# MihailMihov/simd-raytracer

Hardware: AMD Instinct MI355X
Metric: Mrays/s (intersect invocations per second), hw09/scene5 dragon 1920x1080 1spp (higher is better)
Workload: dtype f32; 1 GPU; BASELINE configs[1]: scenes/hw09/scene5.crtscene 1920x1080 1spp max_ray_depth=5 (primary + shadow + reflection rays), kd_tree_simd_accel semantics; rays_per_frame=2726485, primary_rays=2073600, parallelism=bucket-tiles x1

## Files before the change

### simd-raytracer_amd/csrc/api.hip

```cpp
#include <hip/hip_runtime.h>

#include <algorithm>
#include <cmath>
#include <cstdio>
#include <cstdlib>
#include <cstring>
#include <mutex>
#include <new>

#include "kernels.hpp"
#include "stream.hpp"
#include "repack.hpp"
#include "occluded.hpp"
#include "build.hpp"

namespace rtk {

static thread_local std::string g_last_error;
void set_error(const std::string &msg) { g_last_error = msg; }

namespace {

int fail(int code, const std::string &msg) { set_error(msg); return code; }

int hip_fail(hipError_t e, const char *what) {
    set_error(std::string(what) + ": " + hipGetErrorString(e));
    return RTK_ERR_HIP;
}

#define RTK_HIP(call)                                        \
    do {                                                     \
        const hipError_t e_ = (call);                        \
        if (e_ != hipSuccess) return hip_fail(e_, #call);    \
    } while (0)

template <typename T>
int upload(const std::vector<T> &src, T **dst) {
    *dst = nullptr;
    const size_t bytes = (src.empty() ? 1 : src.size()) * sizeof(T);
    RTK_HIP(hipMalloc(reinterpret_cast<void **>(dst), bytes));
    if (!src.empty()) RTK_HIP(hipMemcpy(*dst, src.data(), src.size() * sizeof(T), hipMemcpyHostToDevice));
    return RTK_OK;
}

}
}

struct rtk_knobs {
    uint32_t slice_min_tris = rtk::kSliceMinTrisDefault;
    bool shadow_exit = true;
    bool skip_unlit_shadow = true;
    bool bundle_cull = true;
    bool auto_trials = true;
    bool cost_feedback = true;
    unsigned resort_every = 16;
    uint32_t light_cycles = 140000u;
    uint32_t order_floor_cycles = 20000u;
    bool batch_scalar_surv = false;
    bool stream_scalar_surv = true;
    bool repack = true;
    bool raster_tiles = true;
    int repack_skip_bits = 6;
    bool repack_full_bounds = false;
    int repack_skip_bits2 = 14;
    bool repack_dirs3 = false;
    int repack_trace = -1;
    size_t group8_below = 9000;
    int stream_node_factor = 0;
    int stream_deep_level = 99, stream_deep_mode = RTK_TRACE_AUTO;
    uint32_t auto_min_lanes = 12;
    int stream_sort_from = -1;
    bool stream_debug = false;
    bool stream_side = true;
    int stream_lanes = 4;
    int stream_slices = 0;
    int stream_batch = 0;
    int stream_mem_gb = 96;
    int stream_side_below = 2;
    bool first_frame_prior = true;
    bool fast_occluders = true;
    bool traversal_fast = false;

    static rtk_knobs from_env() {
        rtk_knobs k;
        auto geti = [](const char *name, long &out) { const char *e = std::getenv(name); if (!e || !*e) return false; out = std::atol(e); return true; };
        long v;
        if (geti("RTK_SLICE_MIN_TRIS", v) && v > 0) k.slice_min_tris = uint32_t(v);
        if (geti("RTK_SHADOW_EARLY_EXIT", v)) k.shadow_exit = v != 0;
        if (geti("RTK_SKIP_UNLIT_SHADOW", v)) k.skip_unlit_shadow = v != 0;
        if (geti("RTK_BUNDLE_CULL", v)) k.bundle_cull = v != 0;
        if (geti("RTK_AUTO_TRIALS", v)) k.auto_trials = v != 0;
        if (geti("RTK_COST_FEEDBACK", v)) k.cost_feedback = v != 0;
        if (geti("RTK_COST_RESORT_EVERY", v) && v > 0) k.resort_every = unsigned(v);
        if (geti("RTK_LIGHT_BELOW_CYCLES", v) && v >= 0) k.light_cycles = uint32_t(v);
        if (geti("RTK_ORDER_FLOOR_CYCLES", v) && v >= 0) k.order_floor_cycles = uint32_t(v);
        if (geti("RTK_REPACK", v)) k.repack = v != 0;
        if (geti("RTK_RASTER_TILES", v)) k.raster_tiles = v != 0;
        if (geti("RTK_REPACK_FULL_BOUNDS", v)) k.repack_full_bounds = v != 0;
        if (geti("RTK_REPACK_SKIP_BITS2", v) && v >= 0 && v <= 22) k.repack_skip_bits2 = int(v);
        if (geti("RTK_REPACK_DIRS3", v)) k.repack_dirs3 = v != 0;
        if (geti("RTK_REPACK_SKIP_BITS", v) && v >= 0 && v <= 14) k.repack_skip_bits = int(v);
        if (geti("RTK_STREAM_SCALAR_SURV", v)) k.stream_scalar_surv = v != 0;
        if (geti("RTK_BATCH_SCALAR_SURV", v)) k.batch_scalar_surv = v != 0;
        if (geti("RTK_REPACK_TRACE", v) && (v == RTK_TRACE_AUTO || v == RTK_TRACE_WAVE || v == RTK_TRACE_LANE)) k.repack_trace = int(v);
        if (geti("RTK_GROUP8_BELOW_BLOCKS", v) && v >= 0) k.group8_below = size_t(v);
        if (geti("RTK_STREAM_NODE_FACTOR", v) && v >= 1) k.stream_node_factor = int(v);
        if (geti("RTK_STREAM_DEEP_LEVEL", v)) k.stream_deep_level = int(v);
        if (geti("RTK_STREAM_DEEP_MODE", v)) k.stream_deep_mode = int(v);
        if (geti("RTK_AUTO_MIN_LANES", v) && v > 0 && v <= 64) k.auto_min_lanes = uint32_t(v);
        if (geti("RTK_STREAM_SORT_FROM", v)) k.stream_sort_from = int(v);
        if (geti("RTK_STREAM_DEBUG", v)) k.stream_debug = v != 0;
        if (geti("RTK_STREAM_SIDE", v)) k.stream_side = v != 0;
        if (geti("RTK_TRAVERSAL_FAST", v)) k.traversal_fast = v != 0;
        if (geti("RTK_FIRST_FRAME_PRIOR", v)) k.first_frame_prior = v != 0;
        if (geti("RTK_STREAM_SLICES", v) && (v == 0 || v == 1 || v == 2 || v == 4)) k.stream_slices = int(v);
        if (geti("RTK_STREAM_BATCH", v) && v >= 0 && v <= 4096) k.stream_batch = int(v);
        if (geti("RTK_STREAM_MEM_GB", v) && v >= 1 && v <= 256) k.stream_mem_gb = int(v);
        if (geti("RTK_FAST_OCCLUDERS", v)) k.fast_occluders = v != 0;
        if (geti("RTK_STREAM_SIDE_BELOW", v) && v >= 0) k.stream_side_below = int(v);
        if (geti("RTK_STREAM_LANES", v) && v >= 1 && v <= rtk::dev::kStreamLanes) k.stream_lanes = int(v);
        return k;
    }
// ... 1080 lines not shown
static int render_device_impl(rtk_accel *a, const rtk_render_params *p, float *d_out, hipStream_t s) {
    FrameGeom g;
    int rc = frame_geom(a, p, g);
    if (rc != RTK_OK) return rc;
    if (!d_out) return fail(RTK_ERR_INVALID, "null output buffer");
    dev::RenderArgs A;
    std::memset(&A, 0, sizeof(A));
    A.tree = tree_view(a);
    A.materials = a->d_materials; A.lights = a->d_lights;
    A.textures = a->d_textures; A.tri_uv = a->d_tri_uv; A.tex_pixels = a->d_tex_pixels;
    A.n_lights = int(a->scene.lights.size());
    A.has_refractive = a->has_refractive ? 1 : 0;
    std::memcpy(A.cam_pos, a->scene.cam_pos, sizeof(A.cam_pos));
    std::memcpy(A.cam_mat, a->scene.cam_mat, sizeof(A.cam_mat));
    std::memcpy(A.background, a->scene.background, sizeof(A.background));
    A.width = g.width; A.height = g.height;
    A.aspect = static_cast<float>(g.width) / static_cast<float>(g.height);
    const float fov_radians = static_cast<float>(p->fov_degrees * (3.14159265358979323846 / 180.0));
    A.tan_half_fov = std::tan(fov_radians / 2.0f);
    A.spp = p->spp; A.max_depth = p->max_ray_depth; A.diffuse_rays = p->diffuse_rays; A.seed = p->seed;
    A.width_f = static_cast<float>(g.width); A.height_f = static_cast<float>(g.height);
    A.spp_f = static_cast<float>(p->spp); A.gi_div_f = static_cast<float>(p->diffuse_rays + 1);
    A.sample_begin = g.sample_begin; A.sample_end = g.sample_end;
    A.shadow_bias = p->shadow_bias; A.reflection_bias = p->reflection_bias; A.refraction_bias = p->refraction_bias;
    A.bucket = g.bucket; A.tiles_x = g.tiles_x; A.tiles_y = g.tiles_y; A.n_buckets = g.n_buckets;
    A.blocks_per_bucket_side = g.blocks_side; A.buckets_per_rank = g.buckets_per_rank;
    A.rank = g.rank; A.world = g.world; A.compact = g.world > 1 ? 1 : 0; A.skew_q = g.skew_q;
    A.out = d_out; A.counters = a->d_counters;
    A.slice_min_tris = a->knobs.slice_min_tris;
    const bool forks = a->has_refractive || p->diffuse_rays > 0;
    const bool general = forks || !a->scene.textures.empty();
    A.shadow_exit = (a->knobs.shadow_exit && !a->has_refractive && p->collect_stats != 1) ? 1 : 0;
    A.skip_unlit = (a->knobs.skip_unlit_shadow && !a->has_refractive && p->collect_stats != 1) ? 1 : 0;
    A.occl_on = (a->occl_on && p->collect_stats == 0) ? 1 : 0;
    A.occl = A.tree;
    if (A.occl_on) {
        A.occl.nodes = a->d_occl_nodes; A.occl.leaves = a->d_occl_leaves; A.occl.leaves_fast = nullptr; A.occl.n_leaves = a->occl_n_leaves;
        A.occl.tris = a->d_occl_tris; A.occl.tri_ids = a->d_occl_ids;
    }
    RTK_HIP(hipMemsetAsync(a->d_counters, 0, (kCounterWords + 4) * sizeof(unsigned long long), s));
    if (g.world > 1 && g.sample_begin == 0) {
        size_t nf = size_t(g.buckets_per_rank) * g.bucket * g.bucket * 3;
        RTK_HIP(hipMemsetAsync(d_out, 0, nf * sizeof(float), s));
    }
    bool stream = p->trace_mode == RTK_TRACE_STREAM || (p->trace_mode == RTK_TRACE_AUTO && forks);
    hipEvent_t trial_start = nullptr, trial_end = nullptr;
    if (p->trace_mode == RTK_TRACE_AUTO && forks && !p->collect_stats) {
        const bool trials = a->knobs.auto_trials;
        const uint64_t tsig[3] = {(uint64_t(uint32_t(g.width)) << 32) | uint32_t(g.height), (uint64_t(uint32_t(g.rank)) << 32) | uint32_t(g.world),
                                  (uint64_t(uint32_t(p->spp)) << 32) | (uint64_t(uint32_t(p->max_ray_depth)) << 16) | uint32_t(p->diffuse_rays)};
        if (std::memcmp(tsig, a->trial_sig, sizeof(tsig)) != 0) { std::memcpy(a->trial_sig, tsig, sizeof(tsig)); a->trial_state = 0; }
        if (trials) {
            if (!a->trial_ev[0]) for (auto &e : a->trial_ev) RTK_HIP(hipEventCreate(&e));
            if (a->trial_state == 3) {
                float t_stream = 0.f, t_mega = 0.f;
                if (hipEventQuery(a->trial_ev[1]) == hipSuccess && hipEventQuery(a->trial_ev[3]) == hipSuccess &&
                    hipEventElapsedTime(&t_stream, a->trial_ev[0], a->trial_ev[1]) == hipSuccess &&
                    hipEventElapsedTime(&t_mega, a->trial_ev[2], a->trial_ev[3]) == hipSuccess)
                    a->trial_state = t_mega < t_stream ? 5 : 4;
                else (void)hipGetLastError();
            }
            switch (a->trial_state) {
                case 0: stream = true; trial_start = a->trial_ev[0]; trial_end = a->trial_ev[1]; a->trial_state = 1; break;
                case 1: stream = false; a->trial_state = 2; break;
                case 2: stream = false; trial_start = a->trial_ev[2]; trial_end = a->trial_ev[3]; a->trial_state = 3; break;
                case 5: stream = false; break;
// ... 516 lines not shown
```

### simd-raytracer_amd/csrc/kernels.hip

```cpp
#include <hip/hip_runtime.h>

#include "kernels.hpp"
#include "trace.hip.hpp"
#include "common.hip.hpp"

namespace rtk {
namespace dev {

__device__ __forceinline__ void stage_nodes(const DevNode *g_nodes, uint32_t n_nodes, DevNode *lds_nodes) {
    const float4 *src = reinterpret_cast<const float4 *>(g_nodes);
    float4 *dst = reinterpret_cast<float4 *>(lds_nodes);
    for (uint32_t i = threadIdx.x; i < n_nodes * 2u; i += blockDim.x) dst[i] = src[i];
    __syncthreads();
}

__device__ __forceinline__ void flush_stats(const Stats &st, uint32_t rays, unsigned long long *counters) {
    const uint32_t r = wave_sum(rays), h = wave_sum(st.hits), nd = wave_sum(st.nodes), bp = wave_sum(st.boxpass),
                   lv = wave_sum(st.leaves), tr = wave_sum(st.tris), pk = wave_sum(st.packets16);
    if ((threadIdx.x & 63u) == 0u) {
        atomicAdd(counters + 0, (unsigned long long)r);
        atomicAdd(counters + 2, (unsigned long long)h);
        atomicAdd(counters + 3, (unsigned long long)nd);
        atomicAdd(counters + 4, (unsigned long long)bp);
        atomicAdd(counters + 5, (unsigned long long)lv);
        atomicAdd(counters + 6, (unsigned long long)tr);
        atomicAdd(counters + 7, (unsigned long long)pk);
    }
}

template <int MODE, bool STATS, bool LDS_NODES>
__global__ __launch_bounds__(256) void k_intersect(IntersectArgs A) {
    extern __shared__ __attribute__((aligned(16))) unsigned char smem[];
    DevNode *lds_nodes = reinterpret_cast<DevNode *>(smem);
    if (LDS_NODES) stage_nodes(A.tree.nodes, A.tree.n_nodes, lds_nodes);

    const size_t slot = (size_t)blockIdx.x * blockDim.x + threadIdx.x;
// ... 32 lines not shown
            o0 = make_float4(c.t, c.u, c.v, __uint_as_float(s.tri));
            o1 = make_float4(__uint_as_float(s.mesh), s.hit_normal.x, s.hit_normal.y, s.hit_normal.z);
        } else {
            o0 = make_float4(-1.0f, 0.0f, 0.0f, __uint_as_float(kMiss));
            o1 = make_float4(__uint_as_float(kMiss), 0.0f, 0.0f, 0.0f);
        }
        float4 *out = reinterpret_cast<float4 *>(A.out + i);
        out[0] = o0;
        out[1] = o1;
    }
    if (STATS) flush_stats(st, active ? 1u : 0u, A.counters);
}


__device__ __forceinline__ bool upper_half(const V3 d, const bool sel) {
    Ray q;
    q.o = d; q.d = d; q.inv = d;
    const DirSpread S = dir_spread(q, sel);
    const float dv = S.axis == 0u ? d.x : (S.axis == 1u ? d.y : d.z);
    return sel & !(dv <= S.mid);
}
__device__ __forceinline__ uint32_t burst_part(const V3 d, const bool in, const uint32_t plog) {
    uint32_t part = 0u;
    if (plog == 0u) return part;
    if (upper_half(d, in)) part = 1u;
    if (plog >= 2u) {
#pragma unroll
        for (uint32_t h = 0u; h < 2u; ++h)
            if (upper_half(d, in & (part == h))) part |= 2u;
    }
    return part;
}

template <int SLICES>
struct ShadowBurstService {
    const RenderArgs &A;
    float4 *res;
    __device__ __forceinline__ void operator()(GroupShared *sh, const uint32_t slice) const {
        const uint32_t lane = __lane_id();
        const uint32_t hdr = (uint32_t)__builtin_amdgcn_readfirstlane((int)sh->count);
        const uint32_t plog = hdr & 0xFFu, n_jobs = hdr >> 8;
        const uint32_t first = (uint32_t)__builtin_amdgcn_readfirstlane((int)sh->first);
        const unsigned long long mask = sh->pass_mask;
        const float4 a = sh->ray_o[lane], b = sh->ray_d[lane];
        const V3 P = mk(a.x, a.y, a.z), ncos = mk(a.w, b.x, b.y);
        const bool in_burst = ((mask >> lane) & 1ull) != 0ull;
        for (;;) {
            uint32_t job = 0u;
            if (lane == 0u) job = atomicAdd(&sh->pad[0], 1u);
            job = (uint32_t)__builtin_amdgcn_readfirstlane((int)job);
            if (job >= n_jobs) break;
            const uint32_t k = first + (job >> plog);
            const uint32_t part = job & ((1u << plog) - 1u);
            const float PI_F = 3.14159265358979323846f;
            const DevLight *L = A.lights + k;
            const V3 lp = mk(L->pos[0], L->pos[1], L->pos[2]);
            V3 ld = lp - P;
            const float radius = length(ld);
            const float area = 4.0f * PI_F * radius * radius;
            ld = normalized(ld);
            const float d0 = dot(ld, ncos);
            const float cosine = (0.0f < d0) ? d0 : 0.0f;
            const float contrib = (L->intensity / area) * cosine;
            const bool mine = in_burst & (burst_part(ld, in_burst, plog) == part);
            const bool asked = mine & (0.0f < radius);
            const bool q = asked & !(A.skip_unlit != 0 && unlit_query(contrib, b.z));
            const Ray ray = make_ray(P + (A.shadow_bias * ld), ld);
            Stats st = {0, 0, 0, 0, 0, 0};
            SliceCtx sx = {nullptr, 0xFFFFFFFFu, 0u, true, 0u, group_private_bundles<SLICES>(sh, slice)};
            const float exit_t = A.shadow_exit ? radius : -1.0f;
            const Cand c = trace<RTK_TRACE_WAVE, false, false, 1>(A.tree, nullptr, ray, false, q, st, sx, kAutoMinLanes, exit_t,
                                                                  kClsHasApex | (0x100u + k), lp);
            bool clear = true;
            uint32_t fl = mine ? 2u : 0u;
            if (asked) fl |= 1u;
            if (q) clear = (c.k == kMiss) | (radius < c.t);
            res[job * 64u + lane] = make_float4(contrib, clear ? 1.0f : 0.0f, __uint_as_float(fl), 0.0f);
        }
    }
};

__device__ __forceinline__ uint32_t fresh_lane() {
    uint32_t l;
    asm volatile("v_mbcnt_lo_u32_b32 %0, -1, 0\n\tv_mbcnt_hi_u32_b32 %0, -1, %0" : "=v"(l));
    return l;
}

__device__ __forceinline__ Ray spawn_ray(const V3 o, const V3 d) {
    Ray r;
    r.o = o; r.d = d; r.inv = d;
    return r;
}

enum : int { ST_NEW_SAMPLE = 0, ST_TRACE, ST_SHADE, ST_LIGHT, ST_RETURN, ST_DONE };
enum : int { PEND_CHILD_BG = 0, PEND_CHILD_BLACK = 1, PEND_SHADOW = 2 };
enum : uint32_t { FR_REFR_A = 0, FR_REFR_B = 1, FR_DIFFUSE = 2 };

struct Frame {
    float a[12];
    uint32_t meta;
    uint32_t tri;
    uint32_t key;
};

template <int MODE, bool STATS, bool FORKS, bool LDS_NODES, int SLICES, bool PRIMED = false>
__global__ __launch_bounds__(SLICES > 1 ? 64 * SLICES : 256, SLICES == 16 ? 1 : SLICES == 8 ? 2 : (SLICES == 4 && !STATS ? RTK_G4_WAVES : 4)) void k_render(RenderArgs A) {
#ifdef RTK_DEBUG_PHASES
    const unsigned long long ph_entry = __builtin_readcyclecounter();
    const unsigned long long ph_rt0 = __builtin_amdgcn_s_memrealtime();
#endif
    if (PRIMED && blockIdx.x >= *A.n_listed) return;
    if (A.only_if != nullptr && *A.only_if == 0u) return;
    extern __shared__ __attribute__((aligned(16))) unsigned char smem[];
    DevNode *lds_nodes = reinterpret_cast<DevNode *>(smem);
    constexpr bool kStage = LDS_NODES && (MODE == RTK_TRACE_LANE || MODE == RTK_TRACE_AUTO);
    if (kStage) stage_nodes(A.tree.nodes, A.tree.n_nodes, lds_nodes);
    __shared__ GroupStorage<(SLICES > 1 ? SLICES : 1)> group_st;
    GroupShared *const group_sh = group_st.get();
    const uint32_t wave_in_wg = (uint32_t)__builtin_amdgcn_readfirstlane((int)(threadIdx.x >> 6));
    uint32_t slice = SLICES > 1 ? (wave_in_wg + blockIdx.x) % (uint32_t)SLICES : 0u;
    uint32_t gwave;
    bool light = false;
    if (PRIMED) {
        gwave = A.tile_order[blockIdx.x];
    } else if (SLICES > 1 && A.order_in != nullptr) {
        const uint32_t n_wgs = A.order_hdr[0], n_total = A.order_hdr[1];
        if (blockIdx.x >= n_wgs) return;
        const uint32_t desc = A.wg_list[blockIdx.x];
        if ((desc >> 31) == 0u) {
            gwave = desc;
        } else {
            const uint32_t idx = (desc & 0x7FFFFFFFu) + wave_in_wg;
            if (idx >= n_total) return;
            gwave = A.order_in[idx];
            light = true;
            slice = 0u;
        }
    } else {
        const uint32_t unit = SLICES > 1 ? blockIdx.x : blockIdx.x * (blockDim.x >> 6) + wave_in_wg;
        gwave = (A.order_in != nullptr && unit < A.n_units) ? A.order_in[unit] : unit;
    }
    constexpr int kParkSlots = 4;
    __shared__ __attribute__((aligned(16))) float park_lds[kParkSlots][18][64];
    float4 *const burst_res = reinterpret_cast<float4 *>(&park_lds[1][0][0]);
    constexpr uint32_t kBurstMaxJobs = SLICES > 8 ? 8u : SLICES > 1 ? (uint32_t)SLICES : 1u;
    static_assert(SLICES <= 1 || (size_t)kBurstMaxJobs * 64 * sizeof(float4) <= sizeof(float) * (kParkSlots - 1) * 18 * 64, "burst answers fit the spare parking slots");
    if (SLICES > 1 && slice != 0u) {
        group_helper_loop<SLICES>(A.tree, group_sh, slice, ShadowBurstService<SLICES>{A, burst_res});
        return;
    }
    __shared__ __attribute__((aligned(16))) float wave_bundles[4][kMaxBundles * kBundleFloats];
    SliceCtx sx = {SLICES > 1 ? group_sh : nullptr, light ? 0xFFFFFFFFu : A.slice_min_tris, 0u, true, 0u,
                   (SLICES > 1 && !light) ? group_sh->bundles : wave_bundles[wave_in_wg & 3u]};
    const uint32_t park_slot = (SLICES > 1 && !light) ? 0u : (wave_in_wg & 3u);
    const unsigned long long cost_t0 = __builtin_readcyclecounter();
    const unsigned long long real_t0 = __builtin_amdgcn_s_memrealtime();
    constexpr bool writer = true;
    const uint32_t bpb = A.blocks_per_bucket_side * A.blocks_per_bucket_side;
    const uint32_t local_bucket = gwave / bpb, sub = gwave % bpb;
    const uint32_t bucket = rank_bucket((uint32_t)A.rank, local_bucket, (uint32_t)A.world, A.skew_q);
    bool valid = bucket < A.n_buckets;
    const uint32_t bx = (bucket % A.tiles_x) * A.bucket, by = (bucket / A.tiles_x) * A.bucket;
    const uint32_t sub_x0 = (sub % A.blocks_per_bucket_side) * 8u, sub_y0 = (sub / A.blocks_per_bucket_side) * 8u;
    struct Pixel { uint32_t lx, ly, px, py; };
    const auto my_pixel = [&]() {
        const uint32_t l = fresh_lane();
        Pixel p;
        p.lx = sub_x0 + (l & 7u); p.ly = sub_y0 + (l >> 3);
        p.px = bx + p.lx; p.py = by + p.ly;
        return p;
    };
    {
        const Pixel p = my_pixel();
        valid = valid & (p.lx < A.bucket) & (p.ly < A.bucket) & (p.px < A.width) & (p.py < A.height);
    }

#ifdef RTK_DEBUG_PHASES
    const unsigned long long ph_begin = __builtin_readcyclecounter();
#endif
    const V3 background = mk(A.background[0], A.background[1], A.background[2]);
    const V3 black = mk(0.f, 0.f, 0.f);
    const float PI_F = 3.14159265358979323846f;
    const uint32_t seed_hash = pcg_hash(A.seed);

    int state = valid ? ST_NEW_SAMPLE : ST_DONE;
    int pend = PEND_CHILD_BG;
    int sample = A.sample_begin, depth = 0, light_k = 0;
    uint32_t rkey = 0;
    uint32_t nrays_wave = 0;
    bool cull = false;
    Ray ray = spawn_ray(black, mk(1.f, 1.f, 1.f));
    V3 pixel_sum = black, ret = black;
    if (A.sample_begin > 0 && valid) {
        const Pixel p = my_pixel();
        const float *o = A.out + A.out_index(local_bucket, p.lx, p.ly, p.px, p.py) * 3;
        pixel_sum = mk(o[0], o[1], o[2]);
    }
    V3 P = black, hn = black, fn = black, din = black, ncos = black, acc = black, albedo = black;
    uint32_t hit_tri = 0, hit_mat = 0;
    float shadow_max_t = 0.f, contrib = 0.f;
    bool lit_textured = false;
    Frame frames[FORKS ? kMaxRayDepth : 1];
    int fsp = 0;
    Stats st = {0, 0, 0, 0, 0, 0};
    Cand cand;
    cand.t = kFltMax; cand.u = cand.v = 0.f; cand.k = kMiss;
    bool primed = false;
    V3 mirror_apex = black;
    bool burst_done = false;
    unsigned long long burst_lanes = 0ull;
    uint32_t burst_plog_done = 0u, burst_part0 = 0u;
    uint32_t burst_nl_done = 0u;
#ifdef RTK_DEBUG_PHASES
    unsigned long long ph_first_trace = 0, ph_after_first = 0, ph_wait = 0;
    float ph_tr[6] = {0.f, 0.f, 0.f, 0.f, 0.f, 0.f}, ph_kind[6] = {0.f, 0.f, 0.f, 0.f, 0.f, 0.f};
    float ph_job[3][8] = {{0.f}}, ph_own[1] = {0.f};
#endif

    for (;;) {
        while (state != ST_TRACE && state != ST_DONE) {
            if (state == ST_NEW_SAMPLE) {
                if (sample == A.sample_end) {
                    const float inv = A.spp_f;
                    if (writer) {
                        const Pixel p = my_pixel();
                        float *o = A.out + A.out_index(local_bucket, p.lx, p.ly, p.px, p.py) * 3;
                        if (A.spp == 1 || A.sample_end != A.spp) { o[0] = pixel_sum.x; o[1] = pixel_sum.y; o[2] = pixel_sum.z; }
                        else { o[0] = pixel_sum.x / inv; o[1] = pixel_sum.y / inv; o[2] = pixel_sum.z / inv; }
                    }
                    state = ST_DONE;
                    continue;
                }
                const Pixel p = my_pixel();
                rkey = root_key(seed_hash, p.py * A.width + p.px, (uint32_t)sample);
                ray = camera_ray(A, p.px, p.py, rkey);
                mirror_apex = ray.o;
                cull = true; depth = 0; pend = PEND_CHILD_BG; fsp = 0;
                primed = PRIMED;
                state = ST_TRACE;
            } else if (state == ST_SHADE) {
                if (depth == A.max_depth) { ret = background; state = ST_RETURN; continue; }
                const DevMaterial *mat = A.materials + hit_mat;
                const int kind = mat->kind;
                if (kind == RTK_MAT_CONSTANT) {
                    ret = mk(mat->albedo[0], mat->albedo[1], mat->albedo[2]);
// ... 137 lines not shown
                        cull = false; depth = fdepth + 1; pend = PEND_CHILD_BLACK;
                        state = ST_TRACE;
                    } else {
                        P = fP; hn = fhn;
                        acc = mk(f.a[9], f.a[10], f.a[11]);
                        hit_tri = f.tri;
                        const DevShade *sh = A.tree.shade + hit_tri;
                        fn = mk(sh->fn[0], sh->fn[1], sh->fn[2]);
                        hit_mat = sh->material;
                        const DevMaterial *mat = A.materials + hit_mat;
                        albedo = mk(mat->albedo[0], mat->albedo[1], mat->albedo[2]);
                        ncos = mat->smooth ? hn : fn;
                        lit_textured = false;
                        depth = fdepth;
                        fsp -= 1;
                        light_k = 0;
                        state = ST_LIGHT;
                    }
                }
            }
        }

        const bool need = (state == ST_TRACE);
        if (__ballot(need) == 0ull) break;
        hn = black; fn = black; din = black; ret = black;
        hit_tri = 0u; hit_mat = 0u;
        constexpr bool kRootFirst = !STATS && MODE == RTK_TRACE_WAVE;
        ray.inv = mk((1.0f / ray.d.x), (1.0f / ray.d.y), (1.0f / ray.d.z));
        const float reach = albedo_reach(albedo);
        const bool unlit = (A.skip_unlit != 0) & need & (pend == PEND_SHADOW) && unlit_query(contrib, reach);
        const bool traced = need & !unlit;
        const bool in_root = kRootFirst ? enters_root(A.tree, ray, traced) : traced;
        bool burst = false;
        uint32_t burst_k = 0u, burst_plog = 0u, burst_nl = 0u;
        unsigned long long burst_mask = 0ull;
        bool elsewhere = false;
        uint32_t burst_my_part = 0u;
        if (SLICES > 1 && !STATS && !light && A.has_refractive == 0) {
            const bool sh_lane = need & (pend == PEND_SHADOW);
            burst_mask = __builtin_amdgcn_ballot_w64(sh_lane);
            if (burst_mask != 0ull) {
                burst_k = (uint32_t)__builtin_amdgcn_readlane(light_k, __builtin_ctzll(burst_mask));
                const uint32_t left = (uint32_t)A.n_lights - burst_k;
                burst_nl = left < kBurstMaxJobs ? left : kBurstMaxJobs;
                burst_plog = (burst_nl * 4u <= kBurstMaxJobs) ? 2u : (burst_nl * 2u <= kBurstMaxJobs) ? 1u : 0u;
                burst = (__builtin_amdgcn_ballot_w64(sh_lane & ((uint32_t)light_k != burst_k)) == 0ull) & (1u < (burst_nl << burst_plog));
                if (burst && A.skip_unlit != 0) {
                    bool lit = sh_lane & !unlit;
                    for (uint32_t s = 1u; s < burst_nl; ++s) {
                        const DevLight *L = A.lights + burst_k + s;
                        V3 ld = mk(L->pos[0], L->pos[1], L->pos[2]) - P;
                        const float radius = length(ld);
                        const float area = 4.0f * PI_F * radius * radius;
                        ld = normalized(ld);
                        const float d0 = dot(ld, ncos);
                        const float cosine = (0.0f < d0) ? d0 : 0.0f;
                        lit |= sh_lane & !unlit_query((L->intensity / area) * cosine, reach);
                    }
                    burst = wave_any(lit);
                }
                if (burst) burst_my_part = burst_part(ray.d, sh_lane, burst_plog);
                elsewhere = burst & sh_lane & (burst_my_part != 0u);
            }
        }
        const bool quiet = kRootFirst && !burst && !(PRIMED && wave_any(primed)) && !wave_any(in_root);
        if (quiet) {
            cand.t = kFltMax; cand.u = cand.v = 0.f; cand.k = kMiss;
            burst_done = false;
        } else {
        float *const park = &park_lds[park_slot][0][fresh_lane()];
        park[0 * 64] = pixel_sum.x; park[1 * 64] = pixel_sum.y; park[2 * 64] = pixel_sum.z;
        park[3 * 64] = acc.x; park[4 * 64] = acc.y; park[5 * 64] = acc.z;
        park[6 * 64] = albedo.x; park[7 * 64] = albedo.y; park[8 * 64] = albedo.z;
        park[9 * 64] = ncos.x; park[10 * 64] = ncos.y; park[11 * 64] = ncos.z;
        park[12 * 64] = P.x; park[13 * 64] = P.y; park[14 * 64] = P.z;
        park[15 * 64] = mirror_apex.x; park[16 * 64] = mirror_apex.y; park[17 * 64] = mirror_apex.z;
        if (PRIMED && wave_any(primed)) {
            if (need) {
                const Pixel p = my_pixel();
                const float4 pc = A.prim[A.out_index(local_bucket, p.lx, p.ly, p.px, p.py)];
                cand.t = pc.x; cand.u = pc.y; cand.v = pc.z; cand.k = __float_as_uint(pc.w);
            }
            nrays_wave -= (uint32_t)__popcll(__builtin_amdgcn_ballot_w64(need));
            primed = false;
            burst_done = false;
        } else {
#ifdef RTK_DEBUG_PHASES
            const unsigned long long tr0 = __builtin_readcyclecounter();
            if (ph_first_trace == 0) ph_first_trace = tr0;
#endif
            const float exit_t = (A.shadow_exit && pend == PEND_SHADOW) ? shadow_max_t : -1.0f;
            uint32_t cls = (uint32_t)depth;
            V3 apex = black;
            if (pend == PEND_CHILD_BG) { cls |= kClsHasApex; apex = mirror_apex; }
            if (pend == PEND_SHADOW) {
                const DevLight *L = A.lights + light_k;
                cls = kClsHasApex | (0x100u + (uint32_t)light_k + 0x40u * (uint32_t)depth);
                apex = mk(L->pos[0], L->pos[1], L->pos[2]);
            }
            if (burst) {
                const uint32_t lane = fresh_lane();
                group_sh->ray_o[lane] = make_float4(P.x, P.y, P.z, ncos.x);
                group_sh->ray_d[lane] = make_float4(ncos.y, ncos.z, reach, 0.f);
                if (lane == 0u) {
                    group_sh->pass_mask = burst_mask; group_sh->first = burst_k; group_sh->count = burst_plog | ((burst_nl << burst_plog) << 8);
                    group_sh->pad[0] = 1u;
                    uint32_t extra = GROUP_EXTRA;
                    asm volatile("" : "+v"(extra));
                    group_sh->kind = extra;
                }
                __syncthreads();
                sx.min_tris = 0xFFFFFFFFu;
            }
            cand = trace<MODE, STATS, kStage, SLICES, kRootFirst>(A.tree, lds_nodes, ray, cull, in_root & !elsewhere, st, sx, kAutoMinLanes, exit_t, cls, apex);
#ifdef RTK_DEBUG_PHASES
            const unsigned long long ph_w0 = __builtin_readcyclecounter();
#endif
            if (burst) {
                __syncthreads();
                sx.min_tris = A.slice_min_tris;
            }
#ifdef RTK_DEBUG_PHASES
            ph_wait += __builtin_readcyclecounter() - ph_w0;
            if (burst && SLICES > 1) ph_own[0] = (float)(ph_w0 - tr0);
            for (int i = 0; i < 6; ++i) if (sx.n_trace == (uint32_t)i) {
                ph_tr[i] = (float)(__builtin_readcyclecounter() - tr0);
                ph_kind[i] = burst ? 100.f + (float)burst_plog : (float)__popcll(__builtin_amdgcn_ballot_w64(in_root));
            }
#endif
            burst_done = burst; burst_lanes = burst_mask; burst_plog_done = burst_plog; burst_part0 = burst_my_part;
            burst_nl_done = burst_nl;
#ifdef RTK_DEBUG_PHASES
            sx.c_trace += __builtin_readcyclecounter() - tr0; sx.n_trace += 1u;
            if (ph_after_first == 0) ph_after_first = __builtin_readcyclecounter();
#endif
        }

        float *const unpark = &park_lds[park_slot][0][fresh_lane()];
        pixel_sum = mk(unpark[0 * 64], unpark[1 * 64], unpark[2 * 64]);
        acc = mk(unpark[3 * 64], unpark[4 * 64], unpark[5 * 64]);
        albedo = mk(unpark[6 * 64], unpark[7 * 64], unpark[8 * 64]);
        ncos = mk(unpark[9 * 64], unpark[10 * 64], unpark[11 * 64]);
        P = mk(unpark[12 * 64], unpark[13 * 64], unpark[14 * 64]);
        mirror_apex = mk(unpark[15 * 64], unpark[16 * 64], unpark[17 * 64]);
        }

        uint32_t more_rays = 0u;
        if (need) {
            const uint32_t lane = fresh_lane();
            more_rays = 1u;
            const bool hit = cand.k != kMiss;
            if (pend == PEND_SHADOW) {
                bool clear = !hit | (shadow_max_t < cand.t);
                const bool in_burst = SLICES > 1 && burst_done && ((burst_lanes >> lane) & 1ull) != 0ull;
                const uint32_t my_part = in_burst ? burst_part0 : 0u;
                if (my_part != 0u) clear = burst_res[my_part * 64u + lane].y != 0.0f;
                bool again = false;
                if (!clear && A.has_refractive) {
                    const uint32_t tri = A.tree.tri_ids[cand.k];
                    const uint32_t m = A.tree.shade[tri].material;
                    if (A.materials[m].kind == RTK_MAT_REFRACTIVE) {
                        const V3 hp = ray.o + (cand.t * ray.d);
                        ray.o = hp + (A.shadow_bias * ray.d);
                        shadow_max_t -= cand.t;
                        if (0.0f < shadow_max_t) again = true; else clear = true;
                    }
                }
                if (!again) {
                    if (clear) acc = acc + (contrib * albedo);
                    light_k += 1;
                    state = ST_LIGHT;
                    if (in_burst) {
                        const uint32_t plog = burst_plog_done;
                        for (uint32_t s = 1u; s < burst_nl_done; ++s) {
                            for (uint32_t pp = 0u; pp < (1u << plog); ++pp) {
                                const float4 res = burst_res[((s << plog) + pp) * 64u + lane];
                                const uint32_t fl = __float_as_uint(res.z);
                                if ((fl & 2u) != 0u) {
                                    if (res.y != 0.0f) acc = acc + (res.x * albedo);
                                    more_rays += fl & 1u;
                                }
                            }
                            light_k += 1;
                        }
                    }
                }
            } else if (!hit) {
                ret = (pend == PEND_CHILD_BG) ? background : black;
                state = ST_RETURN;
            } else {
                const Surface s = reconstruct(A.tree, cand);
                P = ray.o + (cand.t * ray.d);
                hn = s.hit_normal; fn = s.face_normal; din = ray.d;
                hit_tri = s.tri; hit_mat = s.material;
                if (FORKS && A.tri_uv != nullptr && A.materials[hit_mat].kind == RTK_MAT_TEXTURE)
                    albedo = sample_texture(A.textures + A.materials[hit_mat].texture, A.tri_uv + hit_tri, cand.u, cand.v, A.tex_pixels);
                state = ST_SHADE;
            }
        }
        nrays_wave += (uint32_t)__popcll(__builtin_amdgcn_ballot_w64((more_rays & 1u) != 0u)) +
                      2u * (uint32_t)__popcll(__builtin_amdgcn_ballot_w64((more_rays & 2u) != 0u)) +
                      4u * (uint32_t)__popcll(__builtin_amdgcn_ballot_w64((more_rays & 4u) != 0u)) +
                      8u * (uint32_t)__popcll(__builtin_amdgcn_ballot_w64((more_rays & 8u) != 0u));
        static_assert(kBurstMaxJobs + 1u <= 15u, "a lane's rays of one iteration fit four bits");
    }

    const uint32_t lane = fresh_lane();
#ifdef RTK_DEBUG_PHASES
    const Pixel dbg_p = my_pixel();
    const uint32_t lx = dbg_p.lx, ly = dbg_p.ly, px = dbg_p.px, py = dbg_p.py;
    if (valid && writer) {
        const unsigned long long ph_now = __builtin_readcyclecounter();
        const unsigned long long ph_rt1 = __builtin_amdgcn_s_memrealtime();
        const float vals[60] = {(float)(ph_now - ph_begin), (float)sx.c_trace, (float)sx.n_trace, (float)sx.n_steps,
                                (float)sx.n_small, (float)sx.t_small, (float)sx.c_small, (float)sx.n_big, (float)sx.t_big, (float)sx.c_big,
// ... 436 lines not shown
```

### simd-raytracer_amd/csrc/kernels.hpp

```cpp
#pragma once

#include <hip/hip_runtime.h>

#include "rtk_internal.hpp"

namespace rtk {

constexpr int kMaxRayDepth = 16;
constexpr int kRayCounterShards = 64;
constexpr int kCriticalWord = 8 + kRayCounterShards;
constexpr unsigned long long kCriticalMinTicks = 1000;
constexpr int kCounterWords = 8 + 2 * kRayCounterShards;
constexpr int kCostBins = 64;
constexpr uint32_t kSliceMinTrisDefault = 33;
constexpr size_t kMaxNodeLdsBytes = 48 * 1024;

}

#include "trace.hip.hpp"

namespace rtk {
namespace dev {

__host__ __device__ inline uint32_t rank_bucket(uint32_t rank, uint32_t local, uint32_t world, uint32_t skew_q) {
// ... 32 lines not shown
    float cam_pos[3];
    float cam_mat[9];
    float background[3];
    uint32_t width, height;
    float aspect;
    float tan_half_fov;
    int spp, max_depth, diffuse_rays;
    int sample_begin, sample_end;
    uint32_t seed;
    float shadow_bias, reflection_bias, refraction_bias;
    uint32_t bucket, tiles_x, tiles_y, n_buckets, blocks_per_bucket_side;
    uint32_t buckets_per_rank;
    uint32_t skew_q;
    int rank, world;
    uint32_t slice_min_tris;
    int compact;
    float *out;
    unsigned long long *counters;
    float4 *prim;
    uint32_t *bin_count;
    uint32_t *bin_list;
    uint32_t *tile_order;
    uint32_t *n_listed;
    uint32_t tile_cap;
    const uint32_t *only_if;
    uint32_t n_units;
    uint32_t *cost_out;
    float width_f, height_f, spp_f, gi_div_f;
    const uint32_t *order_in;
    const uint32_t *order_hdr;
    const uint32_t *wg_list;
    int shadow_exit;
    int skip_unlit;
    int occl_on;
    TreeView occl;

    __device__ __forceinline__ size_t out_index(uint32_t local_bucket, uint32_t lx, uint32_t ly, uint32_t px,
                                                uint32_t py) const {
        return compact ? (((size_t)local_bucket * bucket + ly) * bucket + lx) : ((size_t)py * width + px);
    }
};

struct AssembleArgs {
    const float *gathered;
    float *rgb;
    uint32_t width, height, bucket, tiles_x, world, buckets_per_rank, skew_q;
};

}

hipError_t launch_intersect(const dev::IntersectArgs &A, int mode, bool stats, hipStream_t s);
hipError_t launch_render(const dev::RenderArgs &A, int mode, bool stats, bool forks, hipStream_t s, unsigned n_workgroups = 0);
hipError_t launch_order_by_cost(const uint32_t *cost, uint8_t *bins , uint32_t *order, uint32_t *wg_list ,
                                uint32_t *hdr , uint32_t n, uint32_t light_below, uint32_t floor_below, uint32_t pack,
                                hipStream_t s);
hipError_t launch_block_prior(const dev::RenderArgs &A, uint8_t *cls, uint32_t *order, uint32_t *wg_list, uint32_t *hdr,
                              uint32_t *scratch, uint32_t pack, hipStream_t s);
hipError_t launch_twopass(const dev::RenderArgs &A, bool stats, bool forks, hipStream_t s);
hipError_t launch_assemble(const dev::AssembleArgs &A, hipStream_t s);
hipError_t launch_camera_rays(const dev::RenderArgs &A, int sample, rtk_ray *d_rays, hipStream_t s);
hipError_t launch_to_rgb8(const float *d_rgb, size_t n, uint8_t *d_out, hipStream_t s);

}
```

Before: 14170 Mrays/s.

## Deal shadow burst jobs per light by lit-lane counts via shared table

Reworks the shadow-burst helper protocol. The owning wave now precomputes per-light contributions and lit masks in LDS, then builds a job table where each light gets its own split count. Helper slices pick their light and partition from that table instead of using one uniform split for all lights. The aim is to spend helper jobs only on lights that have lit lanes and to balance the lanes across jobs. In exchange it adds LDS board traffic, per-lane extra light evaluations up front, and more complex job decoding.

New measurement: 14230 Mrays/s (median of 4 runs). Within noise of the previous version (+0.5%).

```diff
diff --git a/simd-raytracer_amd/csrc/api.hip b/simd-raytracer_amd/csrc/api.hip
--- a/simd-raytracer_amd/csrc/api.hip
+++ b/simd-raytracer_amd/csrc/api.hip
@@ -50,6 +50,7 @@
     uint32_t slice_min_tris = rtk::kSliceMinTrisDefault;
     bool shadow_exit = true;
     bool skip_unlit_shadow = true;
+    int burst_deal = 0;
     bool bundle_cull = true;
     bool auto_trials = true;
     bool cost_feedback = true;
@@ -88,6 +89,7 @@
         if (geti("RTK_SLICE_MIN_TRIS", v) && v > 0) k.slice_min_tris = uint32_t(v);
         if (geti("RTK_SHADOW_EARLY_EXIT", v)) k.shadow_exit = v != 0;
         if (geti("RTK_SKIP_UNLIT_SHADOW", v)) k.skip_unlit_shadow = v != 0;
+        if (geti("RTK_BURST_DEAL", v) && v >= 0 && v <= 2) k.burst_deal = int(v);
         if (geti("RTK_BUNDLE_CULL", v)) k.bundle_cull = v != 0;
         if (geti("RTK_AUTO_TRIALS", v)) k.auto_trials = v != 0;
         if (geti("RTK_COST_FEEDBACK", v)) k.cost_feedback = v != 0;
@@ -1234,6 +1236,7 @@
     const bool general = forks || !a->scene.textures.empty();
     A.shadow_exit = (a->knobs.shadow_exit && !a->has_refractive && p->collect_stats != 1) ? 1 : 0;
     A.skip_unlit = (a->knobs.skip_unlit_shadow && !a->has_refractive && p->collect_stats != 1) ? 1 : 0;
+    A.burst_deal = a->knobs.burst_deal;
     A.occl_on = (a->occl_on && p->collect_stats == 0) ? 1 : 0;
     A.occl = A.tree;
     if (A.occl_on) {
diff --git a/simd-raytracer_amd/csrc/burst_deal.hpp b/simd-raytracer_amd/csrc/burst_deal.hpp
--- /dev/null
+++ b/simd-raytracer_amd/csrc/burst_deal.hpp
@@ -0,0 +1,135 @@
+#pragma once
+
+#include <cstdint>
+
+#if defined(__HIPCC__)
+#define RTK_BURST_HD __host__ __device__ __forceinline__
+#define RTK_BURST_UNROLL _Pragma("unroll")
+#else
+#define RTK_BURST_HD inline
+#define RTK_BURST_UNROLL
+#endif
+
+namespace rtk {
+namespace dev {
+
+constexpr uint32_t kBurstMaxLights = 8u;
+constexpr uint32_t kBurstTableCap = 16u;
+enum : uint32_t { BURST_DEAL_BY_LIGHTS = 0u, BURST_DEAL_BY_LIT = 1u, BURST_DEAL_SPLIT_HEAVY = 2u };
+
+struct BurstDeal {
+    uint32_t n_jobs;
+    uint32_t entry[kBurstMaxLights];
+};
+RTK_BURST_HD uint32_t burst_entry_plog(const uint32_t e) { return e & 3u; }
+RTK_BURST_HD uint32_t burst_entry_njobs(const uint32_t e) { return (e >> 2) & 7u; }
+RTK_BURST_HD uint32_t burst_entry_start(const uint32_t e) { return (e >> 5) & 31u; }
+RTK_BURST_HD uint32_t burst_entry_first_part(const uint32_t e) { return (e >> 10) & 1u; }
+
+RTK_BURST_HD uint32_t burst_floor_log2_capped(const uint32_t c) { return c >= 4u ? 2u : (c >= 2u ? 1u : 0u); }
+RTK_BURST_HD uint32_t burst_uniform_plog(const uint32_t n, const uint32_t slices) {
+    return (n * 4u <= slices) ? 2u : ((n * 2u <= slices) ? 1u : 0u);
+}
+
+template <uint32_t MAXL = kBurstMaxLights>
+RTK_BURST_HD BurstDeal burst_deal(const uint32_t (&lit)[MAXL], const uint32_t nl, const uint32_t slices, const uint32_t mode) {
+    static_assert(MAXL <= kBurstMaxLights, "lights of a burst");
+    BurstDeal D;
+    uint32_t cnt[MAXL], plog[MAXL], nj[MAXL], w[MAXL];
+    uint32_t n_lit = 0u, total = 0u;
+RTK_BURST_UNROLL
+    for (uint32_t i = 0u; i < kBurstMaxLights; ++i) D.entry[i] = 0u;
+RTK_BURST_UNROLL
+    for (uint32_t i = 0u; i < MAXL; ++i) {
+        cnt[i] = i < nl ? lit[i] : 0u;
+        n_lit += cnt[i] != 0u ? 1u : 0u;
+        total += cnt[i];
+    }
+    D.n_jobs = 0u;
+    if (n_lit == 0u) return D;
+    const uint32_t p_lights = burst_uniform_plog(nl, slices), p_lit = burst_uniform_plog(n_lit, slices);
+    uint32_t jobs = 0u;
+RTK_BURST_UNROLL
+    for (uint32_t i = 0u; i < MAXL; ++i) {
+        uint32_t p = 0u;
+        if (mode == BURST_DEAL_BY_LIGHTS) {
+            p = p_lights;
+        } else {
+            p = p_lit;
+            if (mode == BURST_DEAL_SPLIT_HEAVY) {
+                uint32_t heavy = (2u * cnt[i] * slices > 5u * total) ? 2u : ((4u * cnt[i] * slices > 5u * total) ? 1u : 0u);
+                if (cnt[i] * n_lit <= total) heavy = 0u;
+                p = p < heavy ? heavy : p;
+            }
+            const uint32_t cap = burst_floor_log2_capped(cnt[i]);
+            p = p < cap ? p : cap;
+        }
+        plog[i] = p;
+        jobs += (i < nl && (mode == BURST_DEAL_BY_LIGHTS || cnt[i] != 0u || i == 0u)) ? (1u << p) : 0u;
+    }
+    const bool overflow = jobs > kBurstTableCap;
+    uint32_t n_jobs = 1u;
+RTK_BURST_UNROLL
+    for (uint32_t i = 0u; i < MAXL; ++i) {
+        if (overflow) {
+            const uint32_t cap = burst_floor_log2_capped(cnt[i]);
+            plog[i] = p_lit < cap ? p_lit : cap;
+        }
+        const bool has = i < nl && (mode == BURST_DEAL_BY_LIGHTS || cnt[i] != 0u);
+        nj[i] = has ? (1u << plog[i]) - (i == 0u ? 1u : 0u) : 0u;
+        w[i] = mode == BURST_DEAL_BY_LIGHTS ? 0u : (cnt[i] >> plog[i]);
+        n_jobs += nj[i];
+    }
+RTK_BURST_UNROLL
+    for (uint32_t i = 0u; i < MAXL; ++i) {
+        uint32_t start = 1u;
+RTK_BURST_UNROLL
+        for (uint32_t j = 0u; j < MAXL; ++j)
+            if (j != i && (w[j] > w[i] || (w[j] == w[i] && j < i))) start += nj[j];
+        D.entry[i] = plog[i] | (nj[i] << 2) | ((nj[i] != 0u ? start : 0u) << 5) | ((i == 0u ? 1u : 0u) << 10);
+    }
+    D.n_jobs = n_jobs;
+    return D;
+}
+
+struct BurstJob { uint32_t light, plog, part; };
+inline uint32_t burst_jobs(const BurstDeal &D, const uint32_t nl, BurstJob (&out)[kBurstTableCap]) {
+    if (D.n_jobs == 0u) return 0u;
+    out[0] = {0u, burst_entry_plog(D.entry[0]), 0u};
+    for (uint32_t i = 0u; i < nl && i < kBurstMaxLights; ++i)
+        for (uint32_t q = 0u; q < burst_entry_njobs(D.entry[i]); ++q)
+            out[burst_entry_start(D.entry[i]) + q] = {i, burst_entry_plog(D.entry[i]), q + burst_entry_first_part(D.entry[i])};
+    return D.n_jobs;
+}
+inline uint64_t burst_upper_half(const float (*d)[3], const uint64_t sel) {
+    const float inf = __builtin_inff();
+    float lo[3] = {inf, inf, inf}, hi[3] = {-inf, -inf, -inf};
+    for (uint32_t l = 0u; l < 64u; ++l)
+        if ((sel >> l) & 1u)
+            for (int a = 0; a < 3; ++a) { lo[a] = d[l][a] < lo[a] ? d[l][a] : lo[a]; hi[a] = hi[a] < d[l][a] ? d[l][a] : hi[a]; }
+    float widest = (hi[0] - lo[0]) * 0.5f, mid = (lo[0] + hi[0]) * 0.5f;
+    int axis = 0;
+    for (int a = 1; a < 3; ++a) {
+        const float wa = (hi[a] - lo[a]) * 0.5f;
+        if (widest < wa) { widest = wa; axis = a; mid = (lo[a] + hi[a]) * 0.5f; }
+    }
+    uint64_t up = 0u;
+    for (uint32_t l = 0u; l < 64u; ++l)
+        if (((sel >> l) & 1u) && !(d[l][axis] <= mid)) up |= uint64_t(1) << l;
+    return up;
+}
+inline void burst_parts(const float (*d)[3], const uint64_t sel, const uint32_t plog, uint32_t (&part)[64]) {
+    uint64_t in[4] = {sel, 0u, 0u, 0u};
+    if (plog >= 1u) { in[1] = burst_upper_half(d, sel); in[0] = sel & ~in[1]; }
+    if (plog >= 2u) {
+        const uint64_t u0 = burst_upper_half(d, in[0]), u1 = burst_upper_half(d, in[1]);
+        in[2] = u0; in[3] = u1; in[0] &= ~u0; in[1] &= ~u1;
+    }
+    for (uint32_t l = 0u; l < 64u; ++l) {
+        part[l] = 0u;
+        for (uint32_t p = 1u; p < 4u; ++p) if ((in[p] >> l) & 1u) part[l] = p;
+    }
+}
+
+}
+}
diff --git a/simd-raytracer_amd/csrc/kernels.hip b/simd-raytracer_amd/csrc/kernels.hip
--- a/simd-raytracer_amd/csrc/kernels.hip
+++ b/simd-raytracer_amd/csrc/kernels.hip
@@ -2,6 +2,7 @@
 
 #include "kernels.hpp"
 #include "trace.hip.hpp"
+#include "burst_deal.hpp"
 #include "common.hip.hpp"
 
 namespace rtk {
@@ -100,50 +101,65 @@
     return part;
 }
 
+constexpr uint32_t kBurstAnswerFloats = kBurstMaxLights * 3u * 64u;
+struct BurstBoard {
+    unsigned long long lit[kBurstMaxLights];
+    uint32_t entry[kBurstMaxLights];
+    unsigned long long lanes;
+    uint32_t n_lights, pad;
+#ifdef RTK_DEBUG_PHASES
+    float job_cycles[kBurstTableCap];
+#endif
+};
 template <int SLICES>
 struct ShadowBurstService {
     const RenderArgs &A;
-    float4 *res;
+    float *res;
+    static constexpr uint32_t kLights = SLICES > 8 ? 8u : (uint32_t)SLICES;
     __device__ __forceinline__ void operator()(GroupShared *sh, const uint32_t slice) const {
         const uint32_t lane = __lane_id();
         const uint32_t hdr = (uint32_t)__builtin_amdgcn_readfirstlane((int)sh->count);
-        const uint32_t plog = hdr & 0xFFu, n_jobs = hdr >> 8;
+        const uint32_t mode = hdr & 0xFFu, n_jobs = hdr >> 8;
         const uint32_t first = (uint32_t)__builtin_amdgcn_readfirstlane((int)sh->first);
         const unsigned long long mask = sh->pass_mask;
-        const float4 a = sh->ray_o[lane], b = sh->ray_d[lane];
-        const V3 P = mk(a.x, a.y, a.z), ncos = mk(a.w, b.x, b.y);
-        const bool in_burst = ((mask >> lane) & 1ull) != 0ull;
+        const BurstBoard *board = reinterpret_cast<const BurstBoard *>(res + kBurstAnswerFloats);
+        const float4 a = sh->ray_o[lane];
+        const V3 P = mk(a.x, a.y, a.z);
+        const uint32_t my_entry = board->entry[lane & (kBurstMaxLights - 1u)];
         for (;;) {
             uint32_t job = 0u;
             if (lane == 0u) job = atomicAdd(&sh->pad[0], 1u);
             job = (uint32_t)__builtin_amdgcn_readfirstlane((int)job);
             if (job >= n_jobs) break;
-            const uint32_t k = first + (job >> plog);
-            const uint32_t part = job & ((1u << plog) - 1u);
-            const float PI_F = 3.14159265358979323846f;
+#ifdef RTK_DEBUG_PHASES
+            const unsigned long long job_t0 = __builtin_readcyclecounter();
+#endif
+            const uint32_t e_start = burst_entry_start(my_entry);
+            const unsigned long long has = __builtin_amdgcn_ballot_w64((lane < kLights) & (e_start <= job) & (job < e_start + burst_entry_njobs(my_entry)));
+            const uint32_t s = (uint32_t)__builtin_ctzll(has | (1ull << 63));
+            const uint32_t e = (uint32_t)__builtin_amdgcn_readlane((int)my_entry, (int)(s & (kBurstMaxLights - 1u)));
+            const uint32_t plog = burst_entry_plog(e), part = job - burst_entry_start(e) + burst_entry_first_part(e);
+            const uint32_t k = first + (s & (kBurstMaxLights - 1u));
             const DevLight *L = A.lights + k;
             const V3 lp = mk(L->pos[0], L->pos[1], L->pos[2]);
             V3 ld = lp - P;
             const float radius = length(ld);
-            const float area = 4.0f * PI_F * radius * radius;
             ld = normalized(ld);
-            const float d0 = dot(ld, ncos);
-            const float cosine = (0.0f < d0) ? d0 : 0.0f;
-            const float contrib = (L->intensity / area) * cosine;
-            const bool mine = in_burst & (burst_part(ld, in_burst, plog) == part);
-            const bool asked = mine & (0.0f < radius);
-            const bool q = asked & !(A.skip_unlit != 0 && unlit_query(contrib, b.z));
+            const unsigned long long lit_mask = board->lit[s & (kBurstMaxLights - 1u)];
+            const bool lit = ((lit_mask >> lane) & 1ull) != 0ull;
+            const bool dom = mode == BURST_DEAL_BY_LIGHTS ? ((mask >> lane) & 1ull) != 0ull : lit;
+            const bool q = lit & dom & (burst_part(ld, dom, plog) == part);
             const Ray ray = make_ray(P + (A.shadow_bias * ld), ld);
             Stats st = {0, 0, 0, 0, 0, 0};
             SliceCtx sx = {nullptr, 0xFFFFFFFFu, 0u, true, 0u, group_private_bundles<SLICES>(sh, slice)};
             const float exit_t = A.shadow_exit ? radius : -1.0f;
             const Cand c = trace<RTK_TRACE_WAVE, false, false, 1>(A.tree, nullptr, ray, false, q, st, sx, kAutoMinLanes, exit_t,
                                                                   kClsHasApex | (0x100u + k), lp);
-            bool clear = true;
-            uint32_t fl = mine ? 2u : 0u;
-            if (asked) fl |= 1u;
-            if (q) clear = (c.k == kMiss) | (radius < c.t);
-            res[job * 64u + lane] = make_float4(contrib, clear ? 1.0f : 0.0f, __uint_as_float(fl), 0.0f);
+            const bool clear = (c.k == kMiss) | (radius < c.t);
+            if (q) res[((s & (kBurstMaxLights - 1u)) * 3u + 1u) * 64u + lane] = clear ? 1.0f : 0.0f;
+#ifdef RTK_DEBUG_PHASES
+            if (lane == 0u) const_cast<BurstBoard *>(board)->job_cycles[job & (kBurstTableCap - 1u)] = (float)(__builtin_readcyclecounter() - job_t0);
+#endif
         }
     }
 };
@@ -210,9 +226,11 @@
     }
     constexpr int kParkSlots = 4;
     __shared__ __attribute__((aligned(16))) float park_lds[kParkSlots][18][64];
-    float4 *const burst_res = reinterpret_cast<float4 *>(&park_lds[1][0][0]);
+    float *const burst_res = &park_lds[1][0][0];
     constexpr uint32_t kBurstMaxJobs = SLICES > 8 ? 8u : SLICES > 1 ? (uint32_t)SLICES : 1u;
-    static_assert(SLICES <= 1 || (size_t)kBurstMaxJobs * 64 * sizeof(float4) <= sizeof(float) * (kParkSlots - 1) * 18 * 64, "burst answers fit the spare parking slots");
+    static_assert(kBurstMaxJobs <= kBurstMaxLights, "a burst's lights fit the table");
+    static_assert((size_t)kBurstAnswerFloats * sizeof(float) + sizeof(BurstBoard) <= sizeof(float) * (kParkSlots - 1) * 18 * 64, "burst answers and table fit the spare parking slots");
+    BurstBoard *const burst_board = reinterpret_cast<BurstBoard *>(burst_res + kBurstAnswerFloats);
     if (SLICES > 1 && slice != 0u) {
         group_helper_loop<SLICES>(A.tree, group_sh, slice, ShadowBurstService<SLICES>{A, burst_res});
         return;
@@ -276,9 +294,6 @@
     bool primed = false;
     V3 mirror_apex = black;
     bool burst_done = false;
-    unsigned long long burst_lanes = 0ull;
-    uint32_t burst_plog_done = 0u, burst_part0 = 0u;
-    uint32_t burst_nl_done = 0u;
 #ifdef RTK_DEBUG_PHASES
     unsigned long long ph_first_trace = 0, ph_after_first = 0, ph_wait = 0;
     float ph_tr[6] = {0.f, 0.f, 0.f, 0.f, 0.f, 0.f}, ph_kind[6] = {0.f, 0.f, 0.f, 0.f, 0.f, 0.f};
@@ -482,10 +497,9 @@
         const bool traced = need & !unlit;
         const bool in_root = kRootFirst ? enters_root(A.tree, ray, traced) : traced;
         bool burst = false;
-        uint32_t burst_k = 0u, burst_plog = 0u, burst_nl = 0u;
+        uint32_t burst_k = 0u, burst_nl = 0u, burst_jobs = 0u;
         unsigned long long burst_mask = 0ull;
         bool elsewhere = false;
-        uint32_t burst_my_part = 0u;
         if (SLICES > 1 && !STATS && !light && A.has_refractive == 0) {
             const bool sh_lane = need & (pend == PEND_SHADOW);
             burst_mask = __builtin_amdgcn_ballot_w64(sh_lane);
@@ -493,24 +507,52 @@
                 burst_k = (uint32_t)__builtin_amdgcn_readlane(light_k, __builtin_ctzll(burst_mask));
                 const uint32_t left = (uint32_t)A.n_lights - burst_k;
                 burst_nl = left < kBurstMaxJobs ? left : kBurstMaxJobs;
-                burst_plog = (burst_nl * 4u <= kBurstMaxJobs) ? 2u : (burst_nl * 2u <= kBurstMaxJobs) ? 1u : 0u;
-                burst = (__builtin_amdgcn_ballot_w64(sh_lane & ((uint32_t)light_k != burst_k)) == 0ull) & (1u < (burst_nl << burst_plog));
-                if (burst && A.skip_unlit != 0) {
-                    bool lit = sh_lane & !unlit;
-                    for (uint32_t s = 1u; s < burst_nl; ++s) {
-                        const DevLight *L = A.lights + burst_k + s;
-                        V3 ld = mk(L->pos[0], L->pos[1], L->pos[2]) - P;
-                        const float radius = length(ld);
-                        const float area = 4.0f * PI_F * radius * radius;
-                        ld = normalized(ld);
-                        const float d0 = dot(ld, ncos);
-                        const float cosine = (0.0f < d0) ? d0 : 0.0f;
-                        lit |= sh_lane & !unlit_query((L->intensity / area) * cosine, reach);
+                if (__builtin_amdgcn_ballot_w64(sh_lane & ((uint32_t)light_k != burst_k)) == 0ull) {
+                    const uint32_t lane = fresh_lane();
+                    uint32_t n_lit[kBurstMaxJobs];
+                    const bool lit0 = sh_lane & !unlit;
+                    const unsigned long long lit0_mask = __builtin_amdgcn_ballot_w64(lit0);
+                    n_lit[0] = (uint32_t)__popcll(lit0_mask);
+                    if (lane == 0u) burst_board->lit[0] = lit0_mask;
+#pragma unroll
+                    for (uint32_t s = 1u; s < kBurstMaxJobs; ++s) {
+                        n_lit[s] = 0u;
+                        if (s < burst_nl) {
+                            const DevLight *L = A.lights + burst_k + s;
+                            V3 ld = mk(L->pos[0], L->pos[1], L->pos[2]) - P;
+                            const float radius = length(ld);
+                            const float area = 4.0f * PI_F * radius * radius;
+                            ld = normalized(ld);
+                            const float d0 = dot(ld, ncos);
+                            const float cosine = (0.0f < d0) ? d0 : 0.0f;
+                            const float c_s = (L->intensity / area) * cosine;
+                            const bool asked = 0.0f < radius;
+                            const unsigned long long m = __builtin_amdgcn_ballot_w64(sh_lane & asked & !((A.skip_unlit != 0) && unlit_query(c_s, reach)));
+                            n_lit[s] = (uint32_t)__popcll(m);
+                            burst_res[(s * 3u + 0u) * 64u + lane] = c_s;
+                            burst_res[(s * 3u + 1u) * 64u + lane] = 1.0f;
+                            burst_res[(s * 3u + 2u) * 64u + lane] = __uint_as_float(asked ? 1u : 0u);
+                            if (lane == 0u) burst_board->lit[s] = m;
+                        }
                     }
-                    burst = wave_any(lit);
+                    const BurstDeal deal = burst_deal<kBurstMaxJobs>(n_lit, burst_nl, kBurstMaxJobs, (uint32_t)A.burst_deal);
+                    burst_jobs = deal.n_jobs;
+                    burst = 1u < burst_jobs;
+                    if (burst) {
+                        if (lane == 0u) {
+#pragma unroll
+                            for (uint32_t s = 0u; s < kBurstMaxJobs; ++s) burst_board->entry[s] = deal.entry[s];
+                            burst_board->lanes = burst_mask; burst_board->n_lights = burst_nl;
+#ifdef RTK_DEBUG_PHASES
+                            for (uint32_t j = 0u; j < kBurstTableCap; ++j) burst_board->job_cycles[j] = 0.f;
+#endif
+                        }
+                        const bool dom = A.burst_deal == (int)BURST_DEAL_BY_LIGHTS ? sh_lane : lit0;
+                        elsewhere = dom & (burst_part(ray.d, dom, burst_entry_plog(deal.entry[0])) != 0u);
+                        burst_res[64u + lane] = 1.0f;
+                        burst_res[128u + lane] = __uint_as_float(elsewhere ? 3u : 1u);
+                    }
                 }
-                if (burst) burst_my_part = burst_part(ray.d, sh_lane, burst_plog);
-                elsewhere = burst & sh_lane & (burst_my_part != 0u);
             }
         }
         const bool quiet = kRootFirst && !burst && !(PRIMED && wave_any(primed)) && !wave_any(in_root);
@@ -550,10 +592,9 @@
             }
             if (burst) {
                 const uint32_t lane = fresh_lane();
-                group_sh->ray_o[lane] = make_float4(P.x, P.y, P.z, ncos.x);
-                group_sh->ray_d[lane] = make_float4(ncos.y, ncos.z, reach, 0.f);
+                group_sh->ray_o[lane] = make_float4(P.x, P.y, P.z, 0.f);
                 if (lane == 0u) {
-                    group_sh->pass_mask = burst_mask; group_sh->first = burst_k; group_sh->count = burst_plog | ((burst_nl << burst_plog) << 8);
+                    group_sh->pass_mask = burst_mask; group_sh->first = burst_k; group_sh->count = (uint32_t)A.burst_deal | (burst_jobs << 8);
                     group_sh->pad[0] = 1u;
                     uint32_t extra = GROUP_EXTRA;
                     asm volatile("" : "+v"(extra));
@@ -572,14 +613,17 @@
             }
 #ifdef RTK_DEBUG_PHASES
             ph_wait += __builtin_readcyclecounter() - ph_w0;
-            if (burst && SLICES > 1) ph_own[0] = (float)(ph_w0 - tr0);
+            if (burst && SLICES > 1 && ph_own[0] <= (float)(__builtin_readcyclecounter() - tr0)) {
+                ph_own[0] = (float)(__builtin_readcyclecounter() - tr0);
+                for (int j = 0; j < 8; ++j) { ph_job[1][j] = burst_board->job_cycles[j]; ph_job[2][j] = burst_board->job_cycles[8 + j]; }
+                ph_job[1][0] = (float)(ph_w0 - tr0);
+            }
             for (int i = 0; i < 6; ++i) if (sx.n_trace == (uint32_t)i) {
                 ph_tr[i] = (float)(__builtin_readcyclecounter() - tr0);
-                ph_kind[i] = burst ? 100.f + (float)burst_plog : (float)__popcll(__builtin_amdgcn_ballot_w64(in_root));
+                ph_kind[i] = burst ? 100.f + (float)burst_jobs : (float)__popcll(__builtin_amdgcn_ballot_w64(in_root));
             }
 #endif
-            burst_done = burst; burst_lanes = burst_mask; burst_plog_done = burst_plog; burst_part0 = burst_my_part;
-            burst_nl_done = burst_nl;
+            burst_done = burst;
 #ifdef RTK_DEBUG_PHASES
             sx.c_trace += __builtin_readcyclecounter() - tr0; sx.n_trace += 1u;
             if (ph_after_first == 0) ph_after_first = __builtin_readcyclecounter();
@@ -602,9 +646,10 @@
             const bool hit = cand.k != kMiss;
             if (pend == PEND_SHADOW) {
                 bool clear = !hit | (shadow_max_t < cand.t);
-                const bool in_burst = SLICES > 1 && burst_done && ((burst_lanes >> lane) & 1ull) != 0ull;
-                const uint32_t my_part = in_burst ? burst_part0 : 0u;
-                if (my_part != 0u) clear = burst_res[my_part * 64u + lane].y != 0.0f;
+                const bool in_burst = SLICES > 1 && burst_done && ((burst_board->lanes >> lane) & 1ull) != 0ull;
+                if (in_burst) {
+                    if ((__float_as_uint(burst_res[128u + lane]) & 2u) != 0u) clear = burst_res[64u + lane] != 0.0f;
+                }
                 bool again = false;
                 if (!clear && A.has_refractive) {
                     const uint32_t tri = A.tree.tri_ids[cand.k];
@@ -621,16 +666,10 @@
                     light_k += 1;
                     state = ST_LIGHT;
                     if (in_burst) {
-                        const uint32_t plog = burst_plog_done;
-                        for (uint32_t s = 1u; s < burst_nl_done; ++s) {
-                            for (uint32_t pp = 0u; pp < (1u << plog); ++pp) {
-                                const float4 res = burst_res[((s << plog) + pp) * 64u + lane];
-                                const uint32_t fl = __float_as_uint(res.z);
-                                if ((fl & 2u) != 0u) {
-                                    if (res.y != 0.0f) acc = acc + (res.x * albedo);
-                                    more_rays += fl & 1u;
-                                }
-                            }
+                        const uint32_t nl_done = burst_board->n_lights;
+                        for (uint32_t s = 1u; s < nl_done; ++s) {
+                            if (burst_res[(s * 3u + 1u) * 64u + lane] != 0.0f) acc = acc + (burst_res[(s * 3u + 0u) * 64u + lane] * albedo);
+                            more_rays += __float_as_uint(burst_res[(s * 3u + 2u) * 64u + lane]) & 1u;
                             light_k += 1;
                         }
                     }
diff --git a/simd-raytracer_amd/csrc/kernels.hpp b/simd-raytracer_amd/csrc/kernels.hpp
--- a/simd-raytracer_amd/csrc/kernels.hpp
+++ b/simd-raytracer_amd/csrc/kernels.hpp
@@ -88,6 +88,7 @@
     const uint32_t *wg_list;
     int shadow_exit;
     int skip_unlit;
+    int burst_deal;
     int occl_on;
     TreeView occl;
 
```
